# swishersnaaake/sexy-raytracer

Hardware: AMD Instinct MI355X
Metric: Msamples/s (WxHxspp/s), 720p masterchief @5k spp (higher is better)
Workload: dtype f32; 1 GPU; masterchief_720p_5000spp; scene=masterchief, width=1280, height=720, spp=5000, max_bounce=4, seed=1, spp_chunks=625, tree=reference, traversal=faithful (bvh.h order), parallelism=tiles8x8 interleaved over 1 rank(s), 1 gather (none)

## Files before the change

sexy-raytracer_amd/csrc/srt_api.cpp:

```cpp

#include <hip/hip_runtime.h>

#include <algorithm>
#include <cstdarg>
#include <cstdio>
#include <cstdlib>
#include <cstring>
#include <string>
#include <vector>

#include "srt_context.h"
#include "srt_launch.h"
#include "srt_regroup.h"
#include "srt_thread.h"

int fail(SrtContext* ctx, const char* fmt, ...) {
  char buf[512];
  va_list ap;
  va_start(ap, fmt);
  vsnprintf(buf, sizeof buf, fmt, ap);
  va_end(ap);
  if (ctx) ctx->error = buf;
  fprintf(stderr, "srt_hip: %s\n", buf);
  return 1;
// ... 35 lines not shown
const TunableName kTunables[] = {
    {"tile_block", nullptr, &Tunables::tileBlock, SRT_TILE_BLOCK},
    {"unit_tiles", "SRT_UNIT_TILES", &Tunables::unitTiles, -1},
    {"queues", "SRT_QUEUES", &Tunables::queues, -1},
    {"shade_min", "SRT_SHADE_MIN", &Tunables::shadeMin, -1},
    {"prim_min", "SRT_PRIM_MIN", &Tunables::primMin, 12},
    {"hit_min", "SRT_HIT_MIN", &Tunables::hitMin, 24},
    {"fuse_min", "SRT_FUSE_MIN", &Tunables::fuseMin, 32},
    {"node_burst", "SRT_NODE_BURST", &Tunables::nodeBurst, -1},
    {"ploc_radius", "SRT_PLOC_RADIUS", &Tunables::plocRadius, 64},
    {"fast_div", "SRT_FAST_DIV", &Tunables::fastDiv, 1},
    {"prim_again_min", "SRT_PRIM_AGAIN_MIN", &Tunables::primAgainMin, 4},
    {"keep_eighths", "SRT_KEEP_EIGHTHS", &Tunables::keepEighths, -1},
    {"chunk_scratch_mb", "SRT_CHUNK_SCRATCH_MB", &Tunables::chunkScratchMb, 12288},
    {"lds_tree", "SRT_LDS_TREE", &Tunables::ldsTree, 1},
    {"wavefront", "SRT_WAVEFRONT", &Tunables::wavefront, 256},
    {"wf_pool", "SRT_WF_POOL", &Tunables::wfPool, 2048},
    {"wf_swap_min", "SRT_WF_SWAP_MIN", &Tunables::wfSwapMin, 0},
    {"wf_swap_big", "SRT_WF_SWAP_BIG", &Tunables::wfSwapBig, 32},
    {"wf_profile", "SRT_WF_PROFILE", &Tunables::wfProfile, 0},
    {"wf_hybrid", "SRT_WF_HYBRID", &Tunables::wfHybrid, 1},
    {"wf_resident_max", "SRT_WF_RESIDENT_MAX", &Tunables::wfResidentMax, 0},
    {"wf_far_rounds", "SRT_WF_FAR_ROUNDS", &Tunables::wfFarRounds, 0},
    {"wf_regroup", "SRT_WF_REGROUP", &Tunables::wfRegroup, 1},
    {"denoise_lds_step", "SRT_DENOISE_LDS_STEP", &Tunables::denoiseLdsStep, 4},
    {"tri_cert", "SRT_TRI_CERT", &Tunables::triCert, 1},
};

float triWMaxFor(const SrtContext* ctx) { return ctx->tun.triCert ? SRT_TRI_W_MAX : 0.0f; }

}

int checkSceneReady(SrtContext* ctx, const char* what) {
  if (!ctx->upload.haveScene) return fail(ctx, "%s: no scene uploaded", what);
  if (ctx->upload.geometryDirty) return fail(ctx, "%s: geometry was updated; call srtRefitScene before anything traverses the scene", what);
  return 0;
}

int buildDeviceTrees(SrtContext* ctx) {
  Upload& up = ctx->upload;
  DevScene& s = up.scene;
  int stackDepth = up.hostStackDepth, bvhDepth = up.hostBvhDepth;
  for (size_t k = 0; k < up.deviceBuilds.size(); ++k) {
    const DeviceBuild& b = up.deviceBuilds[k];
    const int32_t* refs = up.buildRefs[k].get<int32_t>();
    const int n = (int)(up.buildRefs[k].bytes() / sizeof(int32_t));
    int depth = 0;
// ... 4 lines not shown
                                        b.base, &depth);
    if (rc) return fail(ctx, "device BVH build of world item %d failed: %s", b.item, hipGetErrorString((hipError_t)rc));
    stackDepth = std::max(stackDepth, depth);
    bvhDepth = std::max(bvhDepth, depth);
  }
  s.stackDepth = stackDepth;
  up.bvhDepth = bvhDepth;
  return 0;
}

static int srtUploadSceneImpl(SrtContext* ctx, const SrtSceneDesc* d) {
  if (!ctx || !d) return 1;
  HIP_OK(ctx, hipSetDevice(ctx->device));
  ctx->upload = Upload();
  ctx->temporalValid = false;
  std::string err = validateScene(d);
  HostScene h;
  if (err.empty()) err = flattenScene(d, SceneOptions{ctx->tun.wfHybrid, ctx->tun.wfResidentMax, ctx->tun.fastDiv}, h);
  if (!err.empty()) return fail(ctx, "%s", err.c_str());

  DevScene& s = ctx->upload.scene;
  if (!h.nodeThread.empty() && uploadVec(ctx, h.nodeThread, &s.nodeThread)) return 1;
  if (!h.nodesRg.empty() && (uploadVec(ctx, h.nodesRg, &s.nodesRg) || uploadVec(ctx, h.nodeThreadRg, &s.nodeThreadRg))) return 1;
  if (!h.nodesWf.empty() && (uploadVec(ctx, h.nodesWf, &s.nodesWf) || uploadVec(ctx, h.worldWf, &s.worldWf) || uploadVec(ctx, h.primSecond, &s.primSecond))) return 1;
  if (uploadVec(ctx, h.primClass, &s.primClass, 16) || uploadVec(ctx, h.nodeAxis, &s.nodeAxis, 64) || uploadVec(ctx, h.nodes, &s.nodes) ||
      uploadVec(ctx, h.triTest, &s.triTest) || uploadVec(ctx, h.triFast, &s.triFast) || uploadVec(ctx, h.triShade, &s.triShade) || uploadVec(ctx, h.spheres, &s.spheres) ||
      uploadVec(ctx, h.triPrimId, &s.triPrimId) || uploadVec(ctx, h.sphPrimId, &s.sphPrimId) || uploadVec(ctx, h.world, &s.world) ||
      uploadVec(ctx, h.materials, &s.materials) || uploadVec(ctx, h.shadeRecs, &s.shadeRecs) || uploadVec(ctx, h.textures, &s.textures) ||
      uploadVec(ctx, h.texels, &s.texels, 64))
    return 1;
  s.wfResident = h.wfResident;
  s.numPrimClass = (int32_t)h.primClass.size();
  s.numWorld = (int32_t)h.world.size();
  s.stackDepth = h.stackDepth;
  s.numNodes = (int32_t)(h.nodes.size() / 2);
  s.numTris = d->numTriangles;
  s.numSpheres = d->numSpheres;
  s.numMaterials = d->numMaterials;
  s.texelBytes = (int32_t)h.texels.size();
  s.fastDivScene = h.fastDivScene;
  s.boxOrderedScene = h.boxOrderedScene;
  s.triWMax = triWMaxFor(ctx);
  ctx->upload.bvhDepth = h.bvhDepth;
  ctx->upload.hostStackDepth = h.stackDepth;
  ctx->upload.hostBvhDepth = h.bvhDepth;
  ctx->upload.plocRadius = ctx->tun.plocRadius;
// ... 232 lines not shown

int srtTestRegroup(const float* nodes8, int32_t numNodes, const int32_t* world, int32_t numWorld, float* outNodes8) {
  if (!nodes8 || !world || !outNodes8 || numNodes < 0 || numWorld < 0) return -1;
  std::vector<float4> nodes(2 * (size_t)numNodes), out;
  if (numNodes) memcpy(nodes.data(), nodes8, nodes.size() * sizeof(float4));
  if (!srtRegroupNodes(nodes, std::vector<int32_t>(world, world + numWorld), out)) return 0;
  if (numNodes) memcpy(outNodes8, out.data(), out.size() * sizeof(float4));
  return 1;
}
int srtTestGetRegroup(SrtContext* ctx, float* outNodes8, int32_t* outLinks, int32_t capacity, int32_t* count) {
  if (!ctx || !count) return 1;
  if (!ctx->upload.haveScene) return fail(ctx, "srtTestGetRegroup: no scene uploaded");
  const DevScene& s = ctx->upload.scene;
  *count = s.nodesRg ? s.numNodes : 0;
  if (!s.nodesRg || (!outNodes8 && !outLinks)) return 0;
  if (capacity < s.numNodes) return fail(ctx, "srtTestGetRegroup: capacity %d < %d", capacity, s.numNodes);
  HIP_OK(ctx, hipSetDevice(ctx->device));
  HIP_OK(ctx, hipDeviceSynchronize());
  if (outNodes8) HIP_OK(ctx, hipMemcpy(outNodes8, s.nodesRg, (size_t)s.numNodes * 32, hipMemcpyDeviceToHost));
  if (outLinks) HIP_OK(ctx, hipMemcpy(outLinks, s.nodeThreadRg, (size_t)s.numNodes * sizeof(int32_t), hipMemcpyDeviceToHost));
  return 0;
}

int srtTestGetTreeAux(SrtContext* ctx, int32_t item, uint8_t* outAxis, float* outPairs16, int32_t capacity, int32_t* count) {
  if (!ctx || !count) return 1;
  if (!ctx->upload.haveScene) return fail(ctx, "srtTestGetTreeAux: no scene uploaded");
  if (item < 0 || item >= (int32_t)ctx->upload.itemNodes.size()) return fail(ctx, "srtTestGetTreeAux: item %d out of range", item);
  HIP_OK(ctx, hipSetDevice(ctx->device));
  int32_t ref = 0;
  HIP_OK(ctx, hipMemcpy(&ref, ctx->upload.scene.world + item, sizeof ref, hipMemcpyDeviceToHost));
  if (ref < 0) return fail(ctx, "srtTestGetTreeAux: item %d is not a tree", item);
  const auto dt = std::find_if(ctx->upload.deviceBuilds.begin(), ctx->upload.deviceBuilds.end(), [&](const DeviceBuild& b) { return b.item == item; });
  const int32_t base = SRT_NODE_INDEX(ref), n = dt != ctx->upload.deviceBuilds.end() ? dt->count : (int32_t)ctx->upload.itemNodes[item].size();
  if (base + n > ctx->upload.scene.numNodes) return fail(ctx, "srtTestGetTreeAux: item %d lies outside the node array", item);
  *count = n;
  if (!outAxis && !outPairs16) return 0;
  if (capacity < n) return fail(ctx, "srtTestGetTreeAux: capacity %d < %d", capacity, n);
  if (outAxis) HIP_OK(ctx, hipMemcpy(outAxis, ctx->upload.scene.nodeAxis + base, (size_t)n, hipMemcpyDeviceToHost));
  if (outPairs16) HIP_OK(ctx, hipMemcpy(outPairs16, ctx->upload.scene.nodes2 + 4 * (size_t)base, (size_t)n * 64, hipMemcpyDeviceToHost));
  return 0;
}

int srtTestGetSlabScene(SrtContext* ctx, int32_t* out2) {
  if (!ctx || !out2) return 1;
  if (!ctx->upload.haveScene) return fail(ctx, "srtTestGetSlabScene: no scene uploaded");
  out2[0] = ctx->upload.scene.fastDivScene;
// ... 116 lines not shown
```

sexy-raytracer_amd/csrc/srt_device.h:

```cpp
#ifndef SRT_DEVICE_H
#define SRT_DEVICE_H

#include <stdint.h>

#include "../../include/srt_hip.h"
#include "../../include/srt_hip_test.h"

#define SRT_REF_DONE ((int32_t)0x80000000)
#define SRT_NODE_REF(index) ((int32_t)(index) << 5)
#define SRT_NODE_INDEX(ref) ((int32_t)(ref) >> 5)
#define SRT_MAX_NODES (1 << 25)
#define SRT_MAX_QUEUES 64
#define SRT_BLOCK 256
#define SRT_BLOCK_TREE 1024
#define SRT_MAT_INDEX_MASK 0x00ffffff
#define SRT_MAT_TYPE_SHIFT 24
#define SRT_MAT_TEXTURED 4
#define SRT_MAT_FLAGS_SHIFT 28

struct DevMaterial {
  int32_t type;
  int32_t albedoTex, normalTex, metallicTex, roughnessTex;
  float albedo[4];
  float metalness, roughness;
// ... 21 lines not shown
  const uint8_t* nodeAxis;
  const int32_t* nodeThread;
  const uint8_t* primClass;
  int32_t numPrimClass;
  const float4* nodesWf;
  const int32_t* worldWf;
  const int32_t* primSecond;
  int32_t wfResident;
  const int32_t* triPrimId;
  const int32_t* sphPrimId;
  const int32_t* world;
  int32_t numWorld;
  int32_t stackDepth;
  int32_t numNodes, numTris, numSpheres;
  int32_t fastDivScene;
  const DevMaterial* materials;
  const uint4* shadeRecs;
  int32_t numMaterials;
  const DevTexture* textures;
  const uint8_t* texels;
  int32_t texelBytes;
  const float4* nodesRg;
  const int32_t* nodeThreadRg;
};

struct DevCamera {
  float origin[3], lleft[3], horizontal[3], vertical[3], hor[3], vert[3];
  float lensRadius, time0, time1;
};

struct SrtFixedAccum {
  long long r, g, b;
  uint32_t flags;
  uint32_t pad;
};

struct RenderArgs {
  DevScene scene;
  DevCamera cam;
  int32_t imageWidth, imageHeight, tilesX, tilesY, numTiles;
  int32_t spp, maxBounce, sampleFirst;
  uint64_t seed;
  float background[3];
  float tMin;
  int32_t tileFirst, tileStride, numLocalTiles;
  int32_t tileBlock;
// ... 207 lines not shown
```

sexy-raytracer_amd/csrc/srt_regroup.h:

```cpp
#pragma once
#include <hip/hip_runtime.h>

#include <cassert>
#include <cmath>
#include <cstdint>
#include <cstring>
#include <vector>

#include "srt_device.h"
#include "srt_records.h"

namespace srt_regroup_detail {
inline int32_t refOf(const std::vector<float4>& nodes, size_t slot) {
  int32_t r;
  memcpy(&r, &nodes[slot].w, 4);
  return r;
}
inline Box boxOfNode(const std::vector<float4>& nodes, size_t i) {
  return Box{{nodes[2 * i].x, nodes[2 * i].y, nodes[2 * i].z}, {nodes[2 * i + 1].x, nodes[2 * i + 1].y, nodes[2 * i + 1].z}};
}
inline double halfArea(const Box& b) {
  const double x = (double)b.mx[0] - b.mn[0], y = (double)b.mx[1] - b.mn[1], z = (double)b.mx[2] - b.mn[2];
  return x * y + y * z + z * x;
}
inline Box unite(const Box& a, const Box& b) {
  const Box r = surrounding(a, b);
  for (int k = 0; k < 3; ++k) {
    assert(memcmp(&r.mn[k], &a.mn[k], 4) == 0 || memcmp(&r.mn[k], &b.mn[k], 4) == 0);
    assert(memcmp(&r.mx[k], &a.mx[k], 4) == 0 || memcmp(&r.mx[k], &b.mx[k], 4) == 0);
  }
  return r;
}
}
// ... 60 lines not shown
          bestK = k;
        }
      }
      const int32_t left = g.me + 1, right = g.me + 2 * bestK;
      const int32_t lRef = SRT_NODE_REF(left), rRef = SRT_NODE_REF(right);
      float lBits, rBits;
      memcpy(&lBits, &lRef, 4);
      memcpy(&rBits, &rRef, 4);
      out[2 * (size_t)g.me] = make_float4(0.0f, 0.0f, 0.0f, lBits);
      out[2 * (size_t)g.me + 1] = make_float4(0.0f, 0.0f, 0.0f, rBits);
      ranges.push_back(Range{right, g.lo + bestK, g.hi});
      ranges.push_back(Range{left, g.lo, g.lo + bestK});
    }
    for (int32_t i = root + count - 1; i >= root; --i) {
      const int32_t l = refOf(out, 2 * (size_t)i), r = refOf(out, 2 * (size_t)i + 1);
      if (l < 0) continue;
      const Box b = unite(boxOfNode(out, (size_t)SRT_NODE_INDEX(l)), boxOfNode(out, (size_t)SRT_NODE_INDEX(r)));
      out[2 * (size_t)i].x = b.mn[0], out[2 * (size_t)i].y = b.mn[1], out[2 * (size_t)i].z = b.mn[2];
      out[2 * (size_t)i + 1].x = b.mx[0], out[2 * (size_t)i + 1].y = b.mx[1], out[2 * (size_t)i + 1].z = b.mx[2];
    }
  }
  return true;
}
```

sexy-raytracer_amd/csrc/srt_render.cpp:

```cpp

#include <hip/hip_runtime.h>

#include <algorithm>
#include <cstring>
#include <vector>

#include "srt_context.h"
#include "srt_launch.h"
#include "srt_lds_layout.h"

int checkParams(SrtContext* ctx, const SrtRenderParams* p) {
  if (checkSceneReady(ctx, "render")) return 1;
  if (!ctx->haveCamera) return fail(ctx, "render: no camera set");
  if (p->imageWidth < 2 || p->imageHeight < 2) return fail(ctx, "render: image must be at least 2x2 (u,v divide by W-1,H-1)");
  if (p->imageWidth > 65535 * SRT_TILE_W || p->imageHeight > 65535 * SRT_TILE_H) return fail(ctx, "render: image larger than 65535 tiles a side");
  if (p->spp < 1) return fail(ctx, "render: spp must be >= 1");
  if (p->sampleFirst < 0 || (int64_t)p->sampleFirst + p->spp > 0x7fffffff) return fail(ctx, "render: bad sample range");
  if (p->maxBounce < 0 || p->maxBounce > SRT_MAX_BOUNCE) return fail(ctx, "render: maxBounce must be in [0,%d]", SRT_MAX_BOUNCE);
  if (p->tileStride < 1 || p->tileFirst < 0 || p->tileFirst >= p->tileStride) return fail(ctx, "render: bad tile split %d/%d", p->tileFirst, p->tileStride);
  if (p->sppChunks < 0 || p->sppChunks > p->spp) return fail(ctx, "render: sppChunks must be in [0, spp] (0 = library default)");
  return 0;
}

static int tileTableFor(SrtContext* ctx, const SrtRenderParams* p, const RenderArgs& a) {
// ... 51 lines not shown
  const RenderPlan& plan = lp.render;
  RenderArgs a;
  setImageArgs(a, ctx, p);
  if (dList) a.numTiles = a.numLocalTiles = listTiles;
  a.maxBounce = p->maxBounce;
  if (lp.sppChunks < 1) return fail(ctx, "render: sppChunks %d x %d tiles exceeds 2^31 work items", p->sppChunks, a.numTiles);
  if (!lp.fitsLds) return fail(ctx, "render: BVH depth %d needs %zu B of LDS per workgroup", ctx->upload.scene.stackDepth, plan.lds);
  setPlanArgs(a, lp);
  if (!dList && tileTableFor(ctx, p, a)) return 1;
  a.tileXY = dList ? dList : ctx->tileTable.get<const uint32_t>();
  a.queue = ctx->dQueue.get<int32_t>();
  unsigned long long* const stats = !moments && (p->countStats || ctx->tun.wfProfile > 0) ? ctx->dStats.get<unsigned long long>() : nullptr;
  a.stats = stats;
  a.aov = p->countStats ? aov : nullptr;
  a.aovDepth = aovDepth;
  const size_t tilePixels = (size_t)a.numLocalTiles * SRT_TILE_PIXELS;
  a.out = static_cast<float4*>(dAccumTiles);
  a.fix = nullptr;
  if (moments) a.mout = static_cast<float4*>(dMoments);
  a.chunkStride = 0;
  bool scratchPath = false;
  if (a.sppChunks > 1 && chunkSumBuffers(ctx, a, moments, tilePixels, stream, scratchPath)) return 1;
  if (plan.form != SRT_FORM_PATH_POOL || plan.count || ctx->tun.wfRegroup <= 0 || !a.scene.boxOrderedScene) a.scene.nodesRg = nullptr, a.scene.nodeThreadRg = nullptr;
  const bool pathPool = srtFormIsPathPool(plan.form);
  const RenderKernel kernel = pathPool ? srt_render_wf_kernel_for(&plan) : srt_render_kernel_for(&plan);
  if (plan.lds > 64 * 1024)
    HIP_OK(ctx, hipFuncSetAttribute(reinterpret_cast<const void*>(kernel), hipFuncAttributeMaxDynamicSharedMemorySize, (int)plan.lds));
  int perCU = 1;
  if (!pathPool && (hipOccupancyMaxActiveBlocksPerMultiprocessor(&perCU, kernel, plan.block, plan.lds) != hipSuccess || perCU < 1)) perCU = 1;
  const int grid = pathPool ? lp.wfGrid : planGrid(ctx->prop.multiProcessorCount, perCU, a.numWork, plan.block);
  if (pathPool) {
    HIP_OK(ctx, ctx->wfPool.reserve((size_t)grid * lp.wfPoolSize * 128));
    const int hiLevels = std::max(0, p->maxBounce - 4);
    HIP_OK(ctx, ctx->wfAttHi.reserve(std::max<size_t>(16, (size_t)grid * 3 * hiLevels * lp.wfPoolSize * sizeof(float))));
    a.wfPool = ctx->wfPool.get<char>();
    a.wfAttHi = ctx->wfAttHi.get<float>();
    HIP_OK(ctx, hipHostGetDevicePointer((void**)&a.wfError, ctx->dWfError, 0));
  } else if (plan.form == SRT_FORM_LDS_TREE) {
    HIP_OK(ctx, ctx->attScratch.reserve((size_t)srtAttSlots(p->maxBounce) * grid * SRT_BLOCK_TREE * sizeof(float)));
    a.attScratch = ctx->attScratch.get<float>();
  }
  HIP_OK(ctx, hipMemsetAsync(a.queue, 0, sizeof(int32_t) * 16 * a.numQueues, stream));
  if (stats) HIP_OK(ctx, hipMemsetAsync(stats, 0, 96 * sizeof(unsigned long long), stream));
  HIP_OK(ctx, hipEventRecord(ctx->evStart, stream));
  ctx->lastPlan = plan;
  ctx->lastGrid = grid;
// ... 518 lines not shown
```

sexy-raytracer_amd/csrc/srt_scene.cpp:

```cpp

#include "srt_scene.h"

#include <algorithm>
#include <cmath>
#include <cstdarg>
#include <cstdio>
#include <cstring>
#include <limits>
#include <random>

#include "srt_lds_layout.h"
#include "srt_regroup.h"
#include "srt_thread.h"

namespace {

std::mt19937& hostGenerator() {
  static std::mt19937 generator;
  return generator;
}
float hostRandomFloat() {
  static std::uniform_real_distribution<float> distribution(0.0f, 1.0f);
  return distribution(hostGenerator());
}
// ... 408 lines not shown
  h.boxOrderedScene = ordered ? 1 : 0;
  if (h.deviceBuilds.empty() && !h.nodes.empty()) {
    srtThreadLinks16(h.nodes, h.world, d->numTriangles, d->numSpheres, h.nodeThread);
    if (o.wfHybrid > 0) {
      const size_t n = h.nodes.size() / 2;
      const size_t fits = srtWfMaxResidentNodes(SRT_WF_HYBRID_POOL, true);
      const size_t fitsWhole = srtWfMaxWholeTreeNodes();
      const size_t cap = o.wfResidentMax > 0 ? std::min<size_t>(fits, (size_t)o.wfResidentMax) : fits;
      if (n > (o.wfResidentMax > 0 ? cap : fitsWhole))
        h.wfResident = srtHybridRecords(h.nodes, h.world, d->numTriangles, d->numSpheres, cap, h.nodesWf, h.worldWf, h.primSecond, &h.wfIndex);
      if (h.nodesWf.empty()) h.wfIndex.clear();
    }
    if (!h.nodeThread.empty() && h.nodesWf.empty() && !adopted && ordered && h.nodes.size() / 2 <= (size_t)srtWfMaxWholeTreeNodes() &&
        srtRegroupNodes(h.nodes, h.world, h.nodesRg)) {
      srtThreadLinks16(h.nodesRg, h.world, d->numTriangles, d->numSpheres, h.nodeThreadRg);
      bool same = !h.nodeThreadRg.empty();
      for (const float4& v : h.nodesRg) same = same && (!certified || (fastDivOperand(v.x) && fastDivOperand(v.y) && fastDivOperand(v.z)));
      for (size_t i = 0; same && i + 1 < h.nodesRg.size(); i += 2)
        same = srtBoxOrdered(Box{{h.nodesRg[i].x, h.nodesRg[i].y, h.nodesRg[i].z}, {h.nodesRg[i + 1].x, h.nodesRg[i + 1].y, h.nodesRg[i + 1].z}});
      if (!same) {
        h.nodesRg.clear();
        h.nodeThreadRg.clear();
      }
    }
  }
  auto classOf = [&](float word, bool sphere) -> uint8_t {
    const int32_t bits = bitsAs<int32_t>(&word);
    const int type = (bits >> SRT_MAT_TYPE_SHIFT) & 3, flags = (bits >> SRT_MAT_FLAGS_SHIFT) & 3;
    if (type != SRT_MAT_PBR) return 2;
    if (!sphere) return 0;
    return flags ? 2 : 1;
  };
  h.triDevIndex.swap(triDevIndex);
  h.primClass.assign((size_t)2 * std::max(d->numTriangles, d->numSpheres) + 2, 2);
  for (int i = 0; i < d->numTriangles; ++i) h.primClass[(size_t)i << 1] = classOf(h.triShade[4 * (size_t)i + 3].w, false);
  for (int i = 0; i < d->numSpheres; ++i) h.primClass[((size_t)i << 1) | 1] = classOf(h.spheres[3 * (size_t)i + 1].w, true);
  return std::string();
}

extern "C" {

float srtHostRandomFloat(void) { return hostRandomFloat(); }
void srtHostRandomReset(void) { hostGenerator().seed(std::mt19937::default_seed); }

int srtMakeCamera(const SrtCameraParams* in, SrtCamera* out) {
  if (!in || !out) return 1;
// ... 27 lines not shown
```

sexy-raytracer_amd/csrc/srt_scene.h:

```cpp
#pragma once
#include <hip/hip_runtime.h>

#include <cstdint>
#include <string>
#include <vector>

#include "srt_device.h"
#include "srt_records.h"

struct BuildNode {
  Box box;
  int32_t left, right;
  uint8_t axis = 3;
};

struct Builder {
  const SrtSceneDesc* d;
  float time0, time1;
  std::vector<float> sortKey;
  std::vector<int32_t> objects;
  std::vector<BuildNode> nodes;
  int maxPending = 0;

  Box childBox(int32_t ref) const;
// ... 19 lines not shown
  std::vector<int32_t> refs;
};

struct HostTree {
  int32_t item;
  int32_t base, count;
  float time0, time1;
};

struct HostScene {
  std::vector<float4> nodes;
  std::vector<uint8_t> nodeAxis;
  std::vector<int32_t> world;
  std::vector<float4> triTest, triShade, triFast, spheres;
  std::vector<int32_t> triPrimId, sphPrimId;
  std::vector<DevMaterial> materials;
  std::vector<DevTexture> textures;
  std::vector<uint8_t> texels;
  std::vector<uint4> shadeRecs;
  std::vector<uint8_t> primClass;
  std::vector<int32_t> nodeThread;
  std::vector<float4> nodesRg;
  std::vector<int32_t> nodeThreadRg;
  std::vector<float4> nodesWf;
  std::vector<int32_t> worldWf, primSecond;
  int32_t wfResident = 0;
  std::vector<std::vector<SrtBvhNode>> itemNodes;
  std::vector<DeviceBuild> deviceBuilds;
  std::vector<HostTree> hostTrees;
  std::vector<int32_t> triDevIndex;
  std::vector<int32_t> wfIndex;
  int stackDepth = 0, bvhDepth = 0;
  int32_t fastDivScene = 0;
  int32_t boxOrderedScene = 0;
};

std::string flattenScene(const SrtSceneDesc* d, const SceneOptions& o, HostScene& out);
```

sexy-raytracer_amd/csrc/srt_wavefront.hip:

```cpp
#include "srt_path.h"
#include "srt_launch.h"
#include "srt_wf_links.h"
#include "srt_wf_rings.h"
#include "srt_lds_layout.h"

#define WF_BLOCK 1024
#define WF_SET_OF(mask) std::integral_constant<uint32_t, (mask)>()
#define WF_CTX_BYTES 128
#define WF_CTL_LIVE 28
#define WF_CTL_ABORT 29
#define WF_PEND_MISS 0
#define WF_PEND_TERMINAL 2

namespace {
enum { W_NODE = 0, W_PRIM = 1, W_SWAP = 2, W_SERVE = 3 };

__device__ __forceinline__ void bufStore4(Rsrc r, int off, float4 v) {
  u32x4 u;
  u.x = __float_as_uint(v.x); u.y = __float_as_uint(v.y); u.z = __float_as_uint(v.z); u.w = __float_as_uint(v.w);
  __builtin_amdgcn_raw_buffer_store_b128(u, r, off, 0, 0);
}
__device__ __forceinline__ void bufStore1(Rsrc r, int off, uint32_t v) { __builtin_amdgcn_raw_buffer_store_b32(v, r, off, 0, 0); }
typedef float f32x4 __attribute__((ext_vector_type(4)));
typedef __attribute__((address_space(3))) const f32x4 LdsVec4;
// ... 23 lines not shown
  const uint64_t seedMixed = mix64(a.seed);
  const V3 background = ld3(a.background);
  const bool regroup = !HYBRID && !COUNT && sc.nodesRg != nullptr;
  const Rsrc rsNodes = makeRsrc(HYBRID ? sc.nodesWf : (regroup ? sc.nodesRg : sc.nodes), sc.numNodes * 32);
  const Rsrc rsTris = makeRsrc(sc.triTest, HYBRID ? sc.numTris * 48 : 0);
  const Rsrc rsFast = makeRsrc(sc.triFast, HYBRID ? 0 : sc.numTris * 64);
  const Rsrc rsSpheres = makeRsrc(sc.spheres, sc.numSpheres * 48);
  const Rsrc rsTexels = makeRsrc(sc.texels, sc.texelBytes);
  const Rsrc rsClass = makeRsrc(sc.primClass, sc.numPrimClass);
  const Rsrc rsSecond = makeRsrc(sc.primSecond, HYBRID ? sc.numPrimClass * 4 : 0);
  const Rsrc rsPool = makeRsrc(a.wfPool + (size_t)blockIdx.x * POOL * WF_CTX_BYTES, POOL * WF_CTX_BYTES);
  const int hiLevels = a.maxBounce > 4 ? a.maxBounce - 4 : 0;
  const Rsrc rsAttHi = makeRsrc(a.wfAttHi + (size_t)blockIdx.x * 3 * hiLevels * POOL, 3 * hiLevels * POOL * 4);
  const bool singleRoot = SINGLE || sc.numWorld == 1;
  auto worldRef = [&](int k) {
    if (HYBRID) return sc.worldWf[k];
    return srtWfRootWord(sc.world[k]);
  };
  const SrtWfRingGeom ringGeom = {a.wfRingCap, a.wfRingShift, a.wfRingMul3};

  {
    float4* dst = reinterpret_cast<float4*>(ldsTree);
    const int32_t* const threads = regroup ? sc.nodeThreadRg : sc.nodeThread;
    for (int i = threadIdx.x; i < resident * 2; i += WF_BLOCK) {
      float4 v = bufLoad4(rsNodes, 16 * i);
      if (!HYBRID) {
        const int32_t thread = threads[i >> 1];
        v.w = __int_as_float((i & 1) ? srtWfMissWord(thread) : srtWfHitWord(__float_as_int(v.w), thread));
      }
      dst[i] = v;
    }
    for (int i = threadIdx.x; i < WF_CTL_WORDS; i += WF_BLOCK) ctl[i] = 0;
    for (int i = threadIdx.x; i < WF_RINGS * RCAP; i += WF_BLOCK) ringSlots[i] = 0;
    __syncthreads();
    for (int id = threadIdx.x; id < POOL; id += WF_BLOCK) ringSlots[WF_RING_NEWITEM * RCAP + id] = (uint16_t)(id + 1);
    if (threadIdx.x == 0) {
      ctl[WF_CTL_TAIL(WF_RING_NEWITEM)] = POOL;
      ctl[WF_CTL_LIVE] = POOL;
    }
    if (threadIdx.x < 16) ctl[threadIdx.x] = (int)(blockIdx.x % (unsigned)a.numQueues);
    __syncthreads();
  }
  int32_t* const waveQueue = ctl + (threadIdx.x >> 6);
  const int qHome = (int)(blockIdx.x % (unsigned)a.numQueues);
  const int unitItems = a.unitTiles * a.sppChunks * SRT_TILE_PIXELS;
  auto queueEnd = [&](int q) { return (q < a.numUnits ? (a.numUnits - q + a.numQueues - 1) / a.numQueues : 0) * unitItems; };

  auto raiseAbort = [&]() {
    if (__hip_atomic_exchange(&ctl[WF_CTL_ABORT], 1, __ATOMIC_RELAXED, WF_WG) == 0 && a.wfError) atomicAdd(a.wfError, 1);
  };
  auto enqueue = [&](auto set, int ring, int id) {
// ... 689 lines not shown
```

sexy-raytracer_amd/csrc/srt_wf_links.h:

```cpp
#pragma once
#include <hip/hip_runtime.h>
#include <stdint.h>

#include "srt_device.h"

#define SRT_WF_DONE ((int32_t)0x80000000)

SRT_HD inline bool srtWfAtNode(int32_t x) { return x >= 0; }
SRT_HD inline bool srtWfAtPrim(int32_t x) { return (uint32_t)x > (uint32_t)SRT_WF_DONE; }

SRT_HD inline int32_t srtWfLeafWord(int32_t first, int32_t second) {
  const uint32_t hi = second != first ? ((uint32_t)second & 0xffffu) - 1u : 0x8000u;
  return (int32_t)(hi << 16 | ((uint32_t)first & 0xffffu));
}
SRT_HD inline int32_t srtWfHitWord(int32_t left, int32_t thread) {
  if (left >= 0) return left;
  const uint32_t follows = (uint32_t)thread & 0xffffu, after = (uint32_t)thread >> 16;
  return srtWfLeafWord(left, follows != after ? (int32_t)(follows | 0xffff0000u) : left);
}
SRT_HD inline int32_t srtWfMissWord(int32_t thread) {
  const int32_t after = thread >> 16;
  return after >= 0 ? SRT_NODE_REF(after) : SRT_WF_DONE;
}
SRT_HD inline int32_t srtWfRootWord(int32_t ref) { return ref >= 0 ? ref : srtWfLeafWord(ref, ref); }

SRT_HD inline int32_t srtWfLeafFirst(int32_t leaf) { return (int32_t)(int16_t)leaf; }
SRT_HD inline bool srtWfLeafHasSecond(int32_t leaf) { return (uint32_t)leaf >= 0x80010000u; }
SRT_HD inline int32_t srtWfLeafRest(int32_t leaf) { return (int32_t)((((uint32_t)leaf >> 16) | 0x80000000u) + 1u); }
```

sexy-raytracer_amd/hipdev.py:

```python
import ctypes as C
import os

import numpy as np

from . import abi

_HERE = os.path.dirname(os.path.abspath(__file__))
LIB_PATH = os.path.join(_HERE, "csrc", "libsrt_hip.so")
if os.environ.get("SRT_HIP_LIB"):
    LIB_PATH = os.path.abspath(os.environ["SRT_HIP_LIB"])

if not os.path.exists(LIB_PATH):
    raise ImportError("HIP extension not built: %s is missing (run __graft_entry__.build() or "
                      "`make -C sexy-raytracer_amd/csrc`)" % LIB_PATH)

try:
    import torch
except ImportError:
    pass

lib = C.CDLL(LIB_PATH)

EXPORTS = ["srtCreate", "srtDestroy", "srtLastError", "srtMakeCamera", "srtHostRandomFloat", "srtHostRandomReset",
           "srtUploadScene", "srtSetCamera", "srtBuildBvh", "srtGetBvh", "srtGetBvhDepth", "srtNumTiles", "srtNumLocalTiles", "srtDefaultSppChunks", "srtPlanSppChunks",
           "srtRenderTiles", "srtResolveTiles", "srtRenderImage", "srtRenderFeatureTiles", "srtRenderFeatureImage",
           "srtDenoise", "srtRenderDenoisedImage", "srtTraceRays", "srtTraceRaysDevice", "srtOccludedDevice", "srtScatterRays",
           "srtRngKey", "srtCameraRaysDevice", "srtScatterRaysDevice", "srtPathStepDevice",
           "srtCompactPathsScratchBytes", "srtCompactPathsDevice",
           "srtRenderTilesMoments", "srtRenderImageMoments", "srtDenoiseMoments", "srtRenderDenoisedImageMoments",
           "srtRenderAdaptive", "srtRenderAdaptiveImage",
           "srtTemporalAccumulate", "srtRenderTemporalFrame", "srtTemporalReset",
           "srtTemporalReproject", "srtRenderTemporalAdaptive", "srtRenderTemporalAdaptiveFrame",
           "srtRenderFeatureTileList", "srtRenderAdaptiveGuided", "srtRenderAdaptiveDenoisedImage",
           "srtRenderTemporalAdaptiveGuided", "srtRenderTemporalAdaptiveGuidedFrame",
           "srtUpdateTriangles", "srtUpdateSpheres", "srtUpdateTrianglesDevice", "srtUpdateSpheresDevice", "srtRefitScene",
           "srtRebuildScene", "srtGetTreeCost",
           "srtSetMotionTracking", "srtRenderMotionTiles", "srtRenderMotionImage", "srtTemporalAccumulateMotion",
           "srtTemporalReprojectMotion",
           "srtCommGetUniqueId", "srtCommInit", "srtGatherTiles", "srtRenderImageRanks", "srtCommDestroy",
           "srtLastKernelMs", "srtGetStats", "srtDeviceInfo"]
TEST_EXPORTS = ["srtSetTunable", "srtGetTunable", "srtGetShadeProfile", "srtGetWfProfile", "srtGetLaunchInfo", "srtRenderAov",
                "srtScatterRaysForm", "srtTestThreadLinks16", "srtTestHybridRecords", "srtTestGetTreeAux", "srtTestChunkSum",
                "srtTestDenoiseScratch", "srtTestGetTriUndecided", "srtTestGetTriFast", "srtTestTriFastRecord", "srtTestGetSlabScene",
                "srtTestRefinedRcp", "srtTestSlabVisit", "srtTestRegroup", "srtTestGetRegroup"]

_vp = C.c_void_p
lib.srtCreate.argtypes = [C.c_int, C.POINTER(_vp)]
lib.srtDestroy.argtypes = [_vp]
lib.srtLastError.argtypes = [_vp]
lib.srtLastError.restype = C.c_char_p
lib.srtMakeCamera.argtypes = [C.POINTER(abi.SrtCameraParams), C.POINTER(abi.SrtCamera)]
lib.srtHostRandomFloat.restype = C.c_float
lib.srtHostRandomReset.restype = None
lib.srtUploadScene.argtypes = [_vp, C.POINTER(abi.SrtSceneDesc)]
lib.srtSetCamera.argtypes = [_vp, C.POINTER(abi.SrtCamera)]
lib.srtBuildBvh.argtypes = [C.POINTER(abi.SrtSceneDesc), C.c_int32, _vp, C.c_int32, C.POINTER(C.c_int32),
                            C.POINTER(C.c_int32)]
lib.srtGetBvh.argtypes = [_vp, C.c_int32, _vp, C.c_int32, C.POINTER(C.c_int32)]
lib.srtGetBvhDepth.argtypes = [_vp, C.POINTER(C.c_int32)]
lib.srtNumTiles.argtypes = [C.c_int32, C.c_int32]
lib.srtNumTiles.restype = C.c_int32
lib.srtNumLocalTiles.argtypes = [C.c_int32, C.c_int32, C.c_int32]
lib.srtNumLocalTiles.restype = C.c_int32
lib.srtDefaultSppChunks.argtypes = [C.c_int32]
lib.srtDefaultSppChunks.restype = C.c_int32
lib.srtPlanSppChunks.argtypes = [C.c_int32, C.c_int32, C.c_int32, C.c_int32]
lib.srtPlanSppChunks.restype = C.c_int32
# ... 75 lines not shown
lib.srtTestDenoiseScratch.argtypes = [_vp, C.c_int32, C.c_int32] + [C.POINTER(C.c_float)] * 4
lib.srtSetTunable.argtypes = [_vp, C.c_char_p, C.c_int32]
lib.srtGetTunable.argtypes = [_vp, C.c_char_p, C.POINTER(C.c_int32)]
lib.srtGetShadeProfile.argtypes = [_vp, _vp]
lib.srtGetWfProfile.argtypes = [_vp, _vp]
lib.srtGetLaunchInfo.argtypes = [_vp, _vp]
lib.srtTestThreadLinks16.argtypes = [_vp, C.c_int32, _vp, C.c_int32, C.c_int32, C.c_int32, _vp]
lib.srtTestHybridRecords.argtypes = [_vp, C.c_int32, _vp, C.c_int32, C.c_int32, C.c_int32, C.c_int32, _vp, _vp, _vp]
lib.srtTestThreadLinks16.restype = lib.srtTestHybridRecords.restype = C.c_int32
lib.srtTestGetTreeAux.argtypes = [_vp, C.c_int32, C.POINTER(C.c_uint8), C.POINTER(C.c_float), C.c_int32, C.POINTER(C.c_int32)]
if hasattr(lib, "srtTestGetTriUndecided"):
    lib.srtTestGetTriUndecided.argtypes = [_vp, C.POINTER(C.c_uint64)]
    lib.srtTestGetTriFast.argtypes = [_vp, _vp, C.c_int32, C.POINTER(C.c_int32)]
    lib.srtTestTriFastRecord.argtypes = [_vp, _vp]
if hasattr(lib, "srtTestGetSlabScene"):
    lib.srtTestGetSlabScene.argtypes = [_vp, C.POINTER(C.c_int32)]
if hasattr(lib, "srtTestRefinedRcp"):
    lib.srtTestRefinedRcp.argtypes = [_vp, C.c_int64, C.c_int64, C.POINTER(C.c_uint64)]
    lib.srtTestSlabVisit.argtypes = [_vp, C.POINTER(C.c_float), C.c_int32, C.c_float, C.c_int32, C.POINTER(C.c_float)]
if hasattr(lib, "srtTestRegroup"):
    lib.srtTestRegroup.argtypes = [_vp, C.c_int32, _vp, C.c_int32, _vp]
    lib.srtTestRegroup.restype = C.c_int32
    lib.srtTestGetRegroup.argtypes = [_vp, _vp, _vp, C.c_int32, C.POINTER(C.c_int32)]
lib.srtRenderAov.argtypes =[_vp, C.POINTER(abi.SrtRenderParams), C.c_int32, _vp]
lib.srtLastKernelMs.argtypes = [_vp, C.POINTER(C.c_float)]
lib.srtGetStats.argtypes = [_vp, C.POINTER(abi.SrtStats)]
lib.srtDeviceInfo.argtypes = [_vp, C.c_char_p, C.c_int32, C.POINTER(C.c_int32), C.POINTER(C.c_int32)]


class SrtError(RuntimeError):
    pass


def make_camera(params):
    cam = abi.SrtCamera()
    if lib.srtMakeCamera(C.byref(params), C.byref(cam)):
        raise SrtError("srtMakeCamera failed")
    return cam


def rng_key(seed, pixel, sample):
    return int(lib.srtRngKey(int(seed) & (2 ** 64 - 1), int(pixel) & 0xffffffff, int(sample) & 0xffffffff))


def host_random_reset():
    lib.srtHostRandomReset()
# ... 579 lines not shown

    def tri_fast_records(self):
        n = C.c_int32(0)
        self._check(lib.srtTestGetTriFast(self.h, None, 0, C.byref(n)))
        out = np.zeros((n.value, 16), np.float32)
        if n.value:
            self._check(lib.srtTestGetTriFast(self.h, out.ctypes.data, n.value, C.byref(n)))
        return out

    def slab_scene(self):
        out = (C.c_int32 * 2)()
        self._check(lib.srtTestGetSlabScene(self.h, out))
        return int(out[0]), int(out[1])

    def regroup(self):
        n = C.c_int32(0)
        self._check(lib.srtTestGetRegroup(self.h, None, None, 0, C.byref(n)))
        if n.value == 0:
            return None
        nodes, links = np.zeros((n.value, 8), np.float32), np.zeros(n.value, np.int32)
        self._check(lib.srtTestGetRegroup(self.h, nodes.ctypes.data, links.ctypes.data, n.value, C.byref(n)))
        return nodes, links

    def refined_rcp_test(self, first_bits, count):
        out = (C.c_uint64 * 2)()
        self._check(lib.srtTestRefinedRcp(self.h, int(first_bits), int(count), out))
        return float(np.array([out[0]], np.uint64).view(np.float64)[0]), np.array([out[1]], np.uint32).view(np.float32)[0]

    def slab_visit_test(self, cases, t_min, certified_scene=1):
        cases = np.ascontiguousarray(cases, np.float32)
        if cases.ndim != 2 or cases.shape[1] != 13:
            raise ValueError("cases must be (n, 13)")
        out = np.zeros((len(cases), 8), np.float32)
        fp = C.POINTER(C.c_float)
        self._check(lib.srtTestSlabVisit(self.h, cases.ctypes.data_as(fp), len(cases), float(t_min), int(certified_scene), out.ctypes.data_as(fp)))
        return out

    def set_tunable(self, name, value):
        self._check(lib.srtSetTunable(self.h, name.encode(), int(value)))

    def get_tunable(self, name):
        v = C.c_int32(0)
        self._check(lib.srtGetTunable(self.h, name.encode(), C.byref(v)))
        return v.value

    def render_aov(self, params, depth=0):
# ... 51 lines not shown
```

Baseline: 6638 Msamples/s.

## Collapse regrouped BVH into SAH-pruned stackless walk sequence for wavefront traversal

Adds a host pass that elides interior BVH nodes whose surface-area cost test says they are not worth visiting, and emits a compacted stackless walk sequence with hit and miss links plus per-item entry words. The wavefront kernel builds its LDS tree from these records when regroup mode 2 is active, and mode 2 becomes the default. The aim is fewer node visits per ray and a smaller resident tree. Eliding nodes turns some binary splits into longer linear runs of siblings, which could cost extra box tests on rays that would otherwise have culled them early.

```diff
diff --git a/sexy-raytracer_amd/csrc/srt_api.cpp b/sexy-raytracer_amd/csrc/srt_api.cpp
--- a/sexy-raytracer_amd/csrc/srt_api.cpp
+++ b/sexy-raytracer_amd/csrc/srt_api.cpp
@@ -81,7 +81,7 @@
     {"wf_hybrid", "SRT_WF_HYBRID", &Tunables::wfHybrid, 1},
     {"wf_resident_max", "SRT_WF_RESIDENT_MAX", &Tunables::wfResidentMax, 0},
     {"wf_far_rounds", "SRT_WF_FAR_ROUNDS", &Tunables::wfFarRounds, 0},
-    {"wf_regroup", "SRT_WF_REGROUP", &Tunables::wfRegroup, 1},
+    {"wf_regroup", "SRT_WF_REGROUP", &Tunables::wfRegroup, 2},
     {"denoise_lds_step", "SRT_DENOISE_LDS_STEP", &Tunables::denoiseLdsStep, 4},
     {"tri_cert", "SRT_TRI_CERT", &Tunables::triCert, 1},
 };
@@ -132,6 +132,8 @@
   DevScene& s = ctx->upload.scene;
   if (!h.nodeThread.empty() && uploadVec(ctx, h.nodeThread, &s.nodeThread)) return 1;
   if (!h.nodesRg.empty() && (uploadVec(ctx, h.nodesRg, &s.nodesRg) || uploadVec(ctx, h.nodeThreadRg, &s.nodeThreadRg))) return 1;
+  if (!h.walkSeq.empty() && uploadVec(ctx, h.walkSeq, &s.walkSeq)) return 1;
+  s.numWalk = h.walkSeq.empty() ? 0 : h.numWalk;
   if (!h.nodesWf.empty() && (uploadVec(ctx, h.nodesWf, &s.nodesWf) || uploadVec(ctx, h.worldWf, &s.worldWf) || uploadVec(ctx, h.primSecond, &s.primSecond))) return 1;
   if (uploadVec(ctx, h.primClass, &s.primClass, 16) || uploadVec(ctx, h.nodeAxis, &s.nodeAxis, 64) || uploadVec(ctx, h.nodes, &s.nodes) ||
       uploadVec(ctx, h.triTest, &s.triTest) || uploadVec(ctx, h.triFast, &s.triFast) || uploadVec(ctx, h.triShade, &s.triShade) || uploadVec(ctx, h.spheres, &s.spheres) ||
@@ -410,6 +412,44 @@
   return 0;
 }
 
+int srtTestRegroupWalk(const float* nodes8, int32_t numNodes, const int32_t* world, int32_t numWorld, uint8_t* outKeep, int32_t* outSrc,
+                       int32_t* outLinks, int32_t* outEntry, int32_t* count) {
+  if (!nodes8 || !world || !outKeep || !outSrc || !outLinks || !outEntry || !count || numNodes < 0 || numWorld < 0) return -1;
+  std::vector<float4> nodes(2 * (size_t)numNodes);
+  if (numNodes) memcpy(nodes.data(), nodes8, nodes.size() * sizeof(float4));
+  SrtRegroupWalk walk;
+  *count = 0;
+  if (!srtRegroupWalk(nodes, std::vector<int32_t>(world, world + numWorld), walk)) return 0;
+  *count = (int32_t)walk.src.size();
+  if (numNodes) memcpy(outKeep, walk.keep.data(), walk.keep.size());
+  if (*count) memcpy(outSrc, walk.src.data(), walk.src.size() * sizeof(int32_t));
+  if (*count) memcpy(outLinks, walk.links.data(), walk.links.size() * sizeof(int32_t));
+  if (numWorld) memcpy(outEntry, walk.entry.data(), walk.entry.size() * sizeof(int32_t));
+  return 1;
+}
+int srtTestGetRegroupWalk(SrtContext* ctx, uint8_t* outKeep, int32_t* outSrc, int32_t* outLinks, int32_t* outEntry, int32_t capacity, int32_t* count) {
+  if (!ctx || !count) return 1;
+  if (!ctx->upload.haveScene) return fail(ctx, "srtTestGetRegroupWalk: no scene uploaded");
+  const DevScene& s = ctx->upload.scene;
+  *count = s.walkSeq ? s.numWalk : 0;
+  if (!s.walkSeq || (!outKeep && !outSrc && !outLinks && !outEntry)) return 0;
+  if (capacity < s.numNodes) return fail(ctx, "srtTestGetRegroupWalk: capacity %d < %d", capacity, s.numNodes);
+  HIP_OK(ctx, hipSetDevice(ctx->device));
+  HIP_OK(ctx, hipDeviceSynchronize());
+  std::vector<int32_t> seq(3 * (size_t)s.numWalk + (size_t)s.numWorld);
+  HIP_OK(ctx, hipMemcpy(seq.data(), s.walkSeq, seq.size() * sizeof(int32_t), hipMemcpyDeviceToHost));
+  if (outKeep) memset(outKeep, 0, (size_t)s.numNodes);
+  for (int32_t j = 0; j < s.numWalk; ++j) {
+    const int32_t src = seq[3 * (size_t)j];
+    if (src < 0 || src >= s.numNodes) return fail(ctx, "srtTestGetRegroupWalk: record %d has source %d", j, src);
+    if (outKeep) outKeep[src] = 1;
+    if (outSrc) outSrc[j] = src;
+    if (outLinks) outLinks[2 * (size_t)j] = seq[3 * (size_t)j + 1], outLinks[2 * (size_t)j + 1] = seq[3 * (size_t)j + 2];
+  }
+  if (outEntry) memcpy(outEntry, seq.data() + 3 * (size_t)s.numWalk, (size_t)s.numWorld * sizeof(int32_t));
+  return 0;
+}
+
 int srtTestGetTreeAux(SrtContext* ctx, int32_t item, uint8_t* outAxis, float* outPairs16, int32_t capacity, int32_t* count) {
   if (!ctx || !count) return 1;
   if (!ctx->upload.haveScene) return fail(ctx, "srtTestGetTreeAux: no scene uploaded");
diff --git a/sexy-raytracer_amd/csrc/srt_device.h b/sexy-raytracer_amd/csrc/srt_device.h
--- a/sexy-raytracer_amd/csrc/srt_device.h
+++ b/sexy-raytracer_amd/csrc/srt_device.h
@@ -67,6 +67,8 @@
   int32_t texelBytes;
   const float4* nodesRg;
   const int32_t* nodeThreadRg;
+  const int32_t* walkSeq;
+  int32_t numWalk;
 };
 
 struct DevCamera {
diff --git a/sexy-raytracer_amd/csrc/srt_regroup.h b/sexy-raytracer_amd/csrc/srt_regroup.h
--- a/sexy-raytracer_amd/csrc/srt_regroup.h
+++ b/sexy-raytracer_amd/csrc/srt_regroup.h
@@ -9,6 +9,7 @@
 
 #include "srt_device.h"
 #include "srt_records.h"
+#include "srt_wf_links.h"
 
 namespace srt_regroup_detail {
 inline int32_t refOf(const std::vector<float4>& nodes, size_t slot) {
@@ -115,3 +116,89 @@
   }
   return true;
 }
+
+struct SrtRegroupWalk {
+  std::vector<uint8_t> keep;
+  std::vector<int32_t> src;
+  std::vector<int32_t> links;
+  std::vector<int32_t> entry;
+};
+
+inline bool srtRegroupWalk(const std::vector<float4>& rg, const std::vector<int32_t>& world, SrtRegroupWalk& out) {
+  using namespace srt_regroup_detail;
+  const size_t n = rg.size() / 2;
+  out = SrtRegroupWalk();
+  auto fail = [&]() { return out = SrtRegroupWalk(), false; };
+  std::vector<uint8_t> keep(n, 0), seen(n, 0);
+  std::vector<int32_t> parent(n, -1), end(n, 0), children(n, 1), count(world.size(), 0), todo;
+  for (size_t wi = 0; wi < world.size(); ++wi) {
+    if (world[wi] < 0) continue;
+    const int32_t root = SRT_NODE_INDEX(world[wi]);
+    todo.assign(1, root);
+    int32_t cnt = 0, last = root;
+    while (!todo.empty()) {
+      const int32_t i = todo.back();
+      todo.pop_back();
+      if (i < 0 || (size_t)i >= n || seen[i]) return fail();
+      seen[i] = 1;
+      cnt++;
+      last = i > last ? i : last;
+      const int32_t l = refOf(rg, 2 * (size_t)i), r = refOf(rg, 2 * (size_t)i + 1);
+      if ((l >= 0) != (r >= 0)) return fail();
+      if (l < 0) continue;
+      const int32_t li = SRT_NODE_INDEX(l), ri = SRT_NODE_INDEX(r);
+      if (li != i + 1 || ri <= li || (size_t)ri >= n) return fail();
+      parent[li] = parent[ri] = i;
+      todo.push_back(ri);
+      todo.push_back(li);
+    }
+    if (last - root + 1 != cnt) return fail();
+    count[wi] = cnt;
+    for (int32_t i = root + cnt - 1; i >= root; --i) {
+      const int32_t l = refOf(rg, 2 * (size_t)i), r = refOf(rg, 2 * (size_t)i + 1);
+      if (l < 0) {
+        keep[i] = 1;
+        end[i] = i + 1;
+        continue;
+      }
+      const int32_t li = SRT_NODE_INDEX(l), ri = SRT_NODE_INDEX(r);
+      if (end[li] != ri) return fail();
+      end[i] = end[ri];
+      const int32_t m = children[li] + children[ri];
+      const bool elide = i == root || halfArea(boxOfNode(rg, (size_t)i)) * (double)m > halfArea(boxOfNode(rg, (size_t)parent[i])) * (double)(m - 1);
+      keep[i] = elide ? 0 : 1;
+      children[i] = elide ? m : 1;
+    }
+  }
+  std::vector<int32_t> number(n + 1, -1);
+  for (size_t i = 0; i < n; ++i)
+    if (keep[i]) {
+      number[i] = (int32_t)out.src.size();
+      out.src.push_back((int32_t)i);
+    }
+  out.links.assign(2 * out.src.size(), SRT_WF_DONE);
+  out.entry.resize(world.size());
+  std::vector<int32_t>& next = end;
+  for (size_t wi = 0; wi < world.size(); ++wi) {
+    if (world[wi] < 0) {
+      out.entry[wi] = srtWfSeqEntryWord(world[wi], -1);
+      continue;
+    }
+    const int32_t root = SRT_NODE_INDEX(world[wi]), stop = root + count[wi];
+    int32_t behind = -1;
+    for (int32_t i = stop - 1; i >= root; --i) {
+      const int32_t e = end[i];
+      const int32_t after = e < stop ? next[e] : -1;
+      if (keep[i]) {
+        const int32_t j = number[i];
+        out.links[2 * (size_t)j] = srtWfSeqHitWord(refOf(rg, 2 * (size_t)i), refOf(rg, 2 * (size_t)i + 1), j);
+        out.links[2 * (size_t)j + 1] = srtWfSeqMissWord(after);
+        behind = j;
+      }
+      next[i] = behind;
+    }
+    out.entry[wi] = srtWfSeqEntryWord(world[wi], next[root]);
+  }
+  out.keep.swap(keep);
+  return true;
+}
diff --git a/sexy-raytracer_amd/csrc/srt_render.cpp b/sexy-raytracer_amd/csrc/srt_render.cpp
--- a/sexy-raytracer_amd/csrc/srt_render.cpp
+++ b/sexy-raytracer_amd/csrc/srt_render.cpp
@@ -97,6 +97,10 @@
   bool scratchPath = false;
   if (a.sppChunks > 1 && chunkSumBuffers(ctx, a, moments, tilePixels, stream, scratchPath)) return 1;
   if (plan.form != SRT_FORM_PATH_POOL || plan.count || ctx->tun.wfRegroup <= 0 || !a.scene.boxOrderedScene) a.scene.nodesRg = nullptr, a.scene.nodeThreadRg = nullptr;
+  if (!a.scene.nodesRg || ctx->tun.wfRegroup < 2 || !a.scene.walkSeq)
+    a.scene.walkSeq = nullptr, a.scene.numWalk = 0;
+  else
+    a.scene.world = a.scene.walkSeq + 3 * (size_t)a.scene.numWalk;
   const bool pathPool = srtFormIsPathPool(plan.form);
   const RenderKernel kernel = pathPool ? srt_render_wf_kernel_for(&plan) : srt_render_kernel_for(&plan);
   if (plan.lds > 64 * 1024)
diff --git a/sexy-raytracer_amd/csrc/srt_scene.cpp b/sexy-raytracer_amd/csrc/srt_scene.cpp
--- a/sexy-raytracer_amd/csrc/srt_scene.cpp
+++ b/sexy-raytracer_amd/csrc/srt_scene.cpp
@@ -454,6 +454,13 @@
         h.nodesRg.clear();
         h.nodeThreadRg.clear();
       }
+      SrtRegroupWalk walk;
+      if (!h.nodesRg.empty() && srtRegroupWalk(h.nodesRg, h.world, walk)) {
+        h.numWalk = (int32_t)walk.src.size();
+        h.walkSeq.reserve(3 * walk.src.size() + walk.entry.size());
+        for (size_t j = 0; j < walk.src.size(); ++j) h.walkSeq.insert(h.walkSeq.end(), {walk.src[j], walk.links[2 * j], walk.links[2 * j + 1]});
+        h.walkSeq.insert(h.walkSeq.end(), walk.entry.begin(), walk.entry.end());
+      }
     }
   }
   auto classOf = [&](float word, bool sphere) -> uint8_t {
diff --git a/sexy-raytracer_amd/csrc/srt_scene.h b/sexy-raytracer_amd/csrc/srt_scene.h
--- a/sexy-raytracer_amd/csrc/srt_scene.h
+++ b/sexy-raytracer_amd/csrc/srt_scene.h
@@ -65,6 +65,8 @@
   std::vector<int32_t> nodeThread;
   std::vector<float4> nodesRg;
   std::vector<int32_t> nodeThreadRg;
+  std::vector<int32_t> walkSeq;
+  int32_t numWalk = 0;
   std::vector<float4> nodesWf;
   std::vector<int32_t> worldWf, primSecond;
   int32_t wfResident = 0;
diff --git a/sexy-raytracer_amd/csrc/srt_wavefront.hip b/sexy-raytracer_amd/csrc/srt_wavefront.hip
--- a/sexy-raytracer_amd/csrc/srt_wavefront.hip
+++ b/sexy-raytracer_amd/csrc/srt_wavefront.hip
@@ -69,11 +69,19 @@
   {
     float4* dst = reinterpret_cast<float4*>(ldsTree);
     const int32_t* const threads = regroup ? sc.nodeThreadRg : sc.nodeThread;
-    for (int i = threadIdx.x; i < resident * 2; i += WF_BLOCK) {
-      float4 v = bufLoad4(rsNodes, 16 * i);
-      if (!HYBRID) {
-        const int32_t thread = threads[i >> 1];
-        v.w = __int_as_float((i & 1) ? srtWfMissWord(thread) : srtWfHitWord(__float_as_int(v.w), thread));
+    const int numSeq = regroup ? sc.numWalk : 0;
+    for (int i = threadIdx.x; i < (numSeq > 0 ? numSeq : resident) * 2; i += WF_BLOCK) {
+      float4 v;
+      if (numSeq > 0) {
+        const int32_t* const rec = sc.walkSeq + 3 * (i >> 1);
+        v = bufLoad4(rsNodes, 32 * rec[0] + 16 * (i & 1));
+        v.w = __int_as_float(rec[1 + (i & 1)]);
+      } else {
+        v = bufLoad4(rsNodes, 16 * i);
+        if (!HYBRID) {
+          const int32_t thread = threads[i >> 1];
+          v.w = __int_as_float((i & 1) ? srtWfMissWord(thread) : srtWfHitWord(__float_as_int(v.w), thread));
+        }
       }
       dst[i] = v;
     }
diff --git a/sexy-raytracer_amd/csrc/srt_wf_links.h b/sexy-raytracer_amd/csrc/srt_wf_links.h
--- a/sexy-raytracer_amd/csrc/srt_wf_links.h
+++ b/sexy-raytracer_amd/csrc/srt_wf_links.h
@@ -27,3 +27,7 @@
 SRT_HD inline int32_t srtWfLeafFirst(int32_t leaf) { return (int32_t)(int16_t)leaf; }
 SRT_HD inline bool srtWfLeafHasSecond(int32_t leaf) { return (uint32_t)leaf >= 0x80010000u; }
 SRT_HD inline int32_t srtWfLeafRest(int32_t leaf) { return (int32_t)((((uint32_t)leaf >> 16) | 0x80000000u) + 1u); }
+
+SRT_HD inline int32_t srtWfSeqHitWord(int32_t left, int32_t right, int32_t j) { return left >= 0 ? SRT_NODE_REF(j + 1) : srtWfLeafWord(left, right); }
+SRT_HD inline int32_t srtWfSeqMissWord(int32_t after) { return after >= 0 ? SRT_NODE_REF(after) : SRT_WF_DONE; }
+SRT_HD inline int32_t srtWfSeqEntryWord(int32_t ref, int32_t first) { return ref >= 0 ? SRT_NODE_REF(first) : srtWfRootWord(ref); }
diff --git a/sexy-raytracer_amd/hipdev.py b/sexy-raytracer_amd/hipdev.py
--- a/sexy-raytracer_amd/hipdev.py
+++ b/sexy-raytracer_amd/hipdev.py
@@ -42,7 +42,8 @@
 TEST_EXPORTS = ["srtSetTunable", "srtGetTunable", "srtGetShadeProfile", "srtGetWfProfile", "srtGetLaunchInfo", "srtRenderAov",
                 "srtScatterRaysForm", "srtTestThreadLinks16", "srtTestHybridRecords", "srtTestGetTreeAux", "srtTestChunkSum",
                 "srtTestDenoiseScratch", "srtTestGetTriUndecided", "srtTestGetTriFast", "srtTestTriFastRecord", "srtTestGetSlabScene",
-                "srtTestRefinedRcp", "srtTestSlabVisit", "srtTestRegroup", "srtTestGetRegroup"]
+                "srtTestRefinedRcp", "srtTestSlabVisit", "srtTestRegroup", "srtTestGetRegroup",
+                "srtTestRegroupWalk", "srtTestGetRegroupWalk"]
 
 _vp = C.c_void_p
 lib.srtCreate.argtypes = [C.c_int, C.POINTER(_vp)]
@@ -164,6 +165,10 @@
     lib.srtTestRegroup.argtypes = [_vp, C.c_int32, _vp, C.c_int32, _vp]
     lib.srtTestRegroup.restype = C.c_int32
     lib.srtTestGetRegroup.argtypes = [_vp, _vp, _vp, C.c_int32, C.POINTER(C.c_int32)]
+if hasattr(lib, "srtTestRegroupWalk"):
+    lib.srtTestRegroupWalk.argtypes = [_vp, C.c_int32, _vp, C.c_int32, _vp, _vp, _vp, _vp, C.POINTER(C.c_int32)]
+    lib.srtTestRegroupWalk.restype = C.c_int32
+    lib.srtTestGetRegroupWalk.argtypes = [_vp, _vp, _vp, _vp, _vp, C.c_int32, C.POINTER(C.c_int32)]
 lib.srtRenderAov.argtypes =[_vp, C.POINTER(abi.SrtRenderParams), C.c_int32, _vp]
 lib.srtLastKernelMs.argtypes = [_vp, C.POINTER(C.c_float)]
 lib.srtGetStats.argtypes = [_vp, C.POINTER(abi.SrtStats)]
@@ -789,6 +794,17 @@
         self._check(lib.srtTestGetRegroup(self.h, nodes.ctypes.data, links.ctypes.data, n.value, C.byref(n)))
         return nodes, links
 
+    def regroup_walk(self):
+        n = C.c_int32(0)
+        self._check(lib.srtTestGetRegroupWalk(self.h, None, None, None, None, 0, C.byref(n)))
+        if n.value == 0:
+            return None
+        nodes = len(self.regroup()[0])
+        keep, src, links = np.zeros(nodes, np.uint8), np.zeros(nodes, np.int32), np.zeros((nodes, 2), np.int32)
+        entry = np.zeros(int(self._scene_keep[1].numWorld), np.int32)
+        self._check(lib.srtTestGetRegroupWalk(self.h, keep.ctypes.data, src.ctypes.data, links.ctypes.data, entry.ctypes.data, nodes, C.byref(n)))
+        return keep, src[:n.value].copy(), links[:n.value].copy(), entry
+
     def refined_rcp_test(self, first_bits, count):
         out = (C.c_uint64 * 2)()
         self._check(lib.srtTestRefinedRcp(self.h, int(first_bits), int(count), out))
```

After: 6971 Msamples/s (median of 6 runs). +5.0%, better.
